# fabian-sp/GGLasso

Hardware: AMD Instinct MI355X
Metric: ADMM iters/sec on (K=32,p=500) GGL at 1/2/4/8 GPUs; eigh HBM GB/s vs peak (higher is better)
Workload: dtype f64

## Files before the change

### gglasso_amd/_lib.py

```python
import ctypes
import os

import numpy as np

_HERE = os.path.dirname(os.path.abspath(__file__))
LIB_PATH = os.path.join(_HERE, "lib", "libggl_hip.so")
DEV_LIB_PATH = os.path.join(_HERE, "lib", "libggl_hip_dev.so")

REG_SGL, REG_GGL, REG_FGL, REG_FSGL = 0, 1, 2, 3
EIG_AUTO, EIG_JACOBI, EIG_ROCSOLVER, EIG_NEWTON_SCHULZ = 0, 1, 2, 3
CTX_STREAM_GIVEN = 1 << 16
OPTIONS = {"speculate": 1, "spec_factor": 2, "ns_mode": 3, "ns_degrees": 4, "theta_flat": 5, "rank_eig": 6, "parts": 7,
           "parts_max_tiles": 8, "symm_variant": 9, "spin_wait": 10, "fused_bounds": 11, "pipeline": 12, "fused_start": 13, "parts_small": 14, "ns_tol": 15, "cw_warm": 16, "chain": 17, "rank_l0_coarse": 18, "isolate": 19, "rank_deflate": 20, "rank_l0_deflate": 21, "fused_cw": 22, "omega_lds": 23, "early_part": 24, "part_priority": 25, "fused_w": 26, "rank_cw": 27, "bound_side": 28, "lds_pinned": 29, "join_flag": 30, "cw_rider": 31, "copy_rider": 32, "reduce_rider": 33, "parts_bias": 34, "parts_order": 35, "download_threads": 36, "group_sched": 37, "omega_poly": 38}


def eig_flags(method=EIG_AUTO, ns_mode=0, ns_degrees=0):
    return int(method) | ((int(ns_mode) & 0x3) << 8) | ((int(ns_degrees) & 0xf) << 12)

JACOBI_MAX_P = 128
NS_MIN_P = 8
BUF_S, BUF_OMEGA, BUF_THETA, BUF_L, BUF_X, BUF_GROUPSQ, BUF_NORMS, BUF_OMEGA_PREV = range(8)
E_ARG, E_HIP, E_SOLVER, E_ALLOC, E_COMM = -1, -2, -3, -4, -5
COV_CENTER, COV_SCALE, COV_TILE32, COV_TILE64 = 1, 2, 4, 8
PHASES = ("form_W", "eig_omega", "recon_omega", "theta", "eig_L", "recon_L", "dual", "reduce", "eig_omega2", "bound",
# ... 89 lines not shown
    "ggl_finalize_L": ([_vp, _i, ctypes.POINTER(_i)], _i),
    "ggl_failed_instances": ([_vp, ctypes.POINTER(_i)], _i),
    "ggl_failed_reason": ([_vp, _i, _dp], _i),
    "ggl_debug_poison": ([_i], _i),
    "ggl_set_odd_dl": ([_i], _i),
    "ggl_reset_instance": ([_vp, _i], _i),
    "ggl_ctx_create_subset": ([_vp, ctypes.POINTER(_i), _i, ctypes.POINTER(_vp)], _i),
    "ggl_get_snapshot_k": ([_vp, _i, _dp, _dp], _i),
    "ggl_get_snapshot_state_k": ([_vp, _i, _dp, _dp], _i),
    "ggl_dev_ns_schedule": ([_d, _i, _i, ctypes.POINTER(_i), _dp, ctypes.POINTER(_i)], _i),
    "ggl_dev_ns_schedule_tol": ([_d, _i, _d, _i, ctypes.POINTER(_i), _dp, ctypes.POINTER(_i)], _i),
    "ggl_dev_group_partition": ([ctypes.POINTER(_i), _i, _i, _i, ctypes.POINTER(_i)], _i),
    "ggl_dev_ns_units": ([_d, _i, _d], _i),
    "ggl_dev_omega_poly_plan": ([_d, _d, _i, ctypes.POINTER(_i), _dp, ctypes.POINTER(_i)], _i),
    "ggl_omega_poly_stats": ([_vp, ctypes.POINTER(ctypes.c_longlong)], _i),
    "ggl_ns_stats": ([_vp, ctypes.POINTER(ctypes.c_longlong)], _i),
    "ggl_rank_stats": ([_vp, ctypes.POINTER(ctypes.c_longlong)], _i),
    "ggl_deflate_stats": ([_vp, ctypes.POINTER(ctypes.c_longlong)], _i),
    "ggl_finalize_stats": ([_vp, ctypes.POINTER(ctypes.c_longlong)], _i),
    "ggl_eig_info": ([_vp, ctypes.POINTER(_i)], _i),
    "ggl_last_dispatch": ([_vp, ctypes.POINTER(ctypes.c_longlong)], _i),
    "ggl_eigh_batched": ([_i, _i, _dp, _dp, _dp, _i], _i),
    "ggl_phiplus": ([_i, _i, _dp, _dp, _dp, _dp], _i),
    "ggl_prox_rank_norm": ([_i, _i, _dp, _dp, _dp, _dp], _i),
    "ggl_phiplus_matrix": ([_i, _i, _dp, _dp, _dp, _i], _i),
    "ggl_rank_matrix": ([_i, _i, _dp, _dp, _dp, _i], _i),
    "ggl_rank_matrix_ex": ([_i, _i, _dp, _dp, _dp, _i, _d, ctypes.POINTER(ctypes.c_longlong)], _i),
    "ggl_rank_matrix_deflate": ([_i, _i, _dp, _dp, _dp, _i, _d, ctypes.POINTER(ctypes.c_longlong)], _i),
    "ggl_prox_od_1norm": ([_i, _dp, _d, _dp, _dp], _i),
    "ggl_prox_p": ([_i, _i, _dp, _d, _d, _i, _dp], _i),
# ... 107 lines not shown
```

### gglasso_amd/build.py

```python
import os
import subprocess
import sys
from concurrent.futures import ThreadPoolExecutor

HERE = os.path.dirname(os.path.abspath(__file__))
CSRC = os.path.join(HERE, "csrc")
LIBDIR = os.path.join(HERE, "lib")
LIB = os.path.join(LIBDIR, "libggl_hip.so")
SOURCES = ["elementwise.hip", "theta_pair.hip", "theta_fsgl.hip", "ext_group.hip", "eig_jacobi.hip", "recon_gemm.hip", "gemm_sym.hip", "covariance.hip", "stars.hip", "kendall.hip", "gemm_i8.hip", "deflate.hip", "omega_lds.hip", "newton_schulz.hip", "ggl_comm.hip", "probes_dev.hip",
           "capi_ctx.hip", "capi_omega.hip", "capi_lstep.hip", "capi_batch.hip", "capi_snapshots.hip", "capi_checks.hip",
           "capi_stats.hip", "capi_comm.hip", "capi_ext.hip", "capi_ops.hip", "capi_data.hip"]
HEADERS = ["common.hpp", "kernels.hpp", "sym_tile.hpp", "ggl_comm.hpp", "capi_internal.hpp", os.path.join("..", "..", "include", "ggl_hip.h")]
HIPCC = os.environ.get("HIPCC", "/opt/rocm/bin/hipcc")
FLAGS = ["--offload-arch=gfx950", "-O3", "-std=c++17", "-fPIC", "-Wall", "-Wno-unused-function",
         "-mllvm", "-amdgpu-mfma-vgpr-form"]


def _stale(target, deps):
    if not os.path.exists(target):
        return True
    t = os.path.getmtime(target)
    return any(os.path.getmtime(d) > t for d in deps)


DEV_LIB = os.path.join(LIBDIR, "libggl_hip_dev.so")


# ... 36 lines not shown
```

### gglasso_amd/csrc/capi_ctx.hip

```cpp
#include "capi_internal.hpp"

static thread_local char g_err[512] = "";

int fail(int code, const char* fmt, ...)
{
    va_list ap;
    va_start(ap, fmt);
    vsnprintf(g_err, sizeof(g_err), fmt, ap);
    va_end(ap);
    return code;
}

void prof_collect(ggl_ctx* c)
{
    if (!c->prof_on) return;
    for (int ph = 0; ph < GGL_NPHASE; ++ph) {
        if (!c->ev_used[ph]) continue;
        float ms = 0.f;
        if (hipEventElapsedTime(&ms, c->ev[ph][0], c->ev[ph][1]) == hipSuccess) {
            c->ph_ms[ph] += ms;
            c->ph_cnt[ph] += 1;
        }
        c->ev_used[ph] = false;
    }
// ... 313 lines not shown
            if (v >= 0 && !symm_variant_built((int)v))
                return fail(GGL_E_ARG, "bad argument: product-kernel variant not in this build");
            c->symm_variant = (int)v;
            break;
        case GGL_OPT_SPIN_WAIT: c->spin_wait = v != 0.0; break;
        case GGL_OPT_FUSED_BOUNDS: c->fused_bounds = v != 0.0; break;
        case GGL_OPT_PIPELINE: c->pipeline = v != 0.0; break;
        case GGL_OPT_FUSED_START: c->fused_start = v != 0.0; break;
        case GGL_OPT_PARTS_SMALL: c->parts_small = (int)v; break;
        case GGL_OPT_GROUP_SCHED:
            if (v != 0.0 && v != 1.0 && v != 2.0 && v != 3.0 && v != 12.0 && v != 13.0)
                return fail(GGL_E_ARG, "bad argument: GGL_OPT_GROUP_SCHED is 0, 1, 2, 3, 12 or 13");
            c->group_sched = (int)v;
            break;
        case GGL_OPT_OMEGA_POLY:
            if (v != 0.0 && v != 1.0) return fail(GGL_E_ARG, "bad argument: GGL_OPT_OMEGA_POLY is 0 or 1");
            c->omega_poly = (int)v;
            break;
#ifdef GGL_DEV
        case GGL_OPT_PARTS_BIAS: c->parts_bias = (int)v; break;
        case GGL_OPT_PARTS_ORDER: c->parts_order = (int)v; break;
        case GGL_OPT_CHAIN: c->chain_mode = (v == 2.0) ? 2 : (v != 0.0 ? 1 : 0); break;
        case GGL_OPT_FUSED_CW: c->fused_cw = v != 0.0; break;
        case GGL_OPT_RANK_CW: c->rank_cw = v != 0.0; break;
        case GGL_OPT_BOUND_SIDE: c->bound_side = (int)v; break;
#else
        case GGL_OPT_PARTS_BIAS: case GGL_OPT_PARTS_ORDER: case GGL_OPT_CHAIN: case GGL_OPT_FUSED_CW: case GGL_OPT_RANK_CW:
        case GGL_OPT_BOUND_SIDE: case GGL_OPT_PART_PRIORITY:
            if (v == 0.0) break;
            return fail(GGL_E_ARG, "bad argument: option %d is a measured-and-rejected alternative that only the development "
                        "library (libggl_hip_dev.so, python -m gglasso_amd.build --dev) carries", opt);
// ... 474 lines not shown
```

### gglasso_amd/csrc/capi_internal.hpp

```cpp
#pragma once
#include <hip/hip_runtime.h>
#include <rocblas/rocblas.h>
#include <rocsolver/rocsolver.h>

#include <algorithm>
#include <cmath>
#include <cstdarg>
#include <cstdio>
#include <cstring>
#include <numeric>
#include <atomic>
#include <thread>
#include <mutex>
#include <chrono>
#include <vector>

#include "../../include/ggl_hip.h"
#include "kernels.hpp"
#include "ggl_comm.hpp"

using namespace ggl;


#define HIPCHK(expr)                                                                                   \
// ... 95 lines not shown
    unsigned long long* join_words = nullptr;
    unsigned long long join_seq = 0;
    hipEvent_t ev_bfork[MAX_PARTS] = {}, ev_bjoin[MAX_PARTS] = {};
    bool pipeline = true, pre_valid = false, pre_spec_pending = false;
    bool last_step_hint = false;
    double* pre_beta = nullptr;
    long long pre_launched = 0, pre_dropped = 0;
    int download_threads = 8;
    GGL_DEV_OPT(int, parts_order);
    GGL_DEV_OPT(int, parts_bias);
    int group_sched = 1;
    long long group_steps = 0;
    long long group_changes = 0;
    int last_groups = 1, last_group_len[MAX_PARTS] = {}, last_group_units[MAX_PARTS] = {};
    double group_units_sum[MAX_PARTS] = {};
    int omega_poly = 1;
    long long poly_seqs = 0, poly_seqs_total = 0;
    int poly_last_deg = 0;
    int parts_small = 8;
    bool fused_start = true;
    bool fused_bounds = true;
    bool lds_omega = true;
    int lds_waves = 0;
    double* lds_tab = nullptr;
    int lds_ntab = 0, lds_tab_deg = -1;
    double lds_lnq = 0.0, lds_tab_tol = -1.0;
    long long lds_calls = 0, lds_misses = 0;
    int lds_cool = 0, lds_cool_next = 4;
    bool lds_last = false;
    GGL_DEV_OPT(bool, fused_cw);
    int theta_flat = 2;
    bool state_symmetric = true;
    bool S_symmetric = false;
// ... 196 lines not shown
```

### gglasso_amd/csrc/capi_omega.hip

```cpp
#include "capi_internal.hpp"

int eig_recon(ggl_ctx* c, double* A, double* out, double* Dv, int map, const double* betaK, int ph_eig,
                     int ph_recon)
{
    c->info_dirty = true;
    if (use_jacobi(c)) {
        if (ph_eig >= 0) PB(c, ph_eig);
        HIPCHK(launch_jacobi(c->stream, A, Dv, nullptr, out, map, betaK, c->info, c->K, c->p));
        if (ph_eig >= 0) PE(c, ph_eig);
        return GGL_OK;
    }
    if (ph_eig >= 0) PB(c, ph_eig);
    {
        int rcb = blas_handle(c, &c->blas);
        if (rcb) return rcb;
    }
    if (c->use_syevj) {
        rocblas_status sj = rocsolver_dsyevj_strided_batched(c->blas, rocblas_esort_none, rocblas_evect_original,
                                                             rocblas_fill_upper, c->p, A, c->p,
                                                             (rocblas_stride)c->p * c->p, 0.0, c->E, 100,
                                                             (rocblas_int*)c->sweeps, Dv, c->p, c->info, c->K);
        if (sj != rocblas_status_success) return fail(GGL_E_SOLVER, "rocsolver_dsyevj_strided_batched: status %d", (int)sj);
        if (ph_eig >= 0) PE(c, ph_eig);
        if (ph_recon >= 0) PB(c, ph_recon);
// ... 196 lines not shown
    t.n += 1;
}
void trace_host(ggl_ctx* c, int tag)
{
    ggl_ctx::Trace& t = c->trace;
    if (!t.on || t.nhost >= t.cap) return;
    t.host_us[t.nhost] = std::chrono::duration<double, std::micro>(std::chrono::steady_clock::now() - t.t0).count();
    t.host_tag[t.nhost] = tag;
    t.nhost += 1;
}
void trace_symm_hook(hipStream_t st, int kind, void* arg) { trace_mark((ggl_ctx*)arg, st, 10 + kind); }

static void note_family(ggl_ctx* c, const NsPlan& pl)
{
    c->poly_seqs_total += 1;
    if (pl.direct) { c->poly_seqs += 1; c->poly_last_deg = pl.direct; }
}

static int omega_groups(const ggl_ctx* c, const double* cb, const double* beta_h, int K, int* Kh, int* k0h, int* gunits)
{
    if (!c->group_sched || K < 2 || c->ns_force == 2 || c->chain_mode || c->comm) return 1;
    {
        const double I = 2.5e-14 * (double)c->p * c->p * c->p, F = 6.5e-6;
        if (c->group_sched < 10 && (double)K * 1e-7 > 0.01 * 7.0 * (F + K * I)) return 1;
    }
    std::vector<int> u(K);
    for (int k = 0; k < K; ++k) {
        double ck = cb[k] * (1.0 + 1e-10);
        if (!(ck > 0.0) || !std::isfinite(ck) || !(beta_h[k] > 0.0)) return 1;
        if (ck < 4.0 * beta_h[k]) ck = 4.0 * beta_h[k];
        u[k] = ns_units_query(std::sqrt(4.0 * beta_h[k] / ck), c->ns_degrees, c->ns_tol);
// ... 1020 lines not shown
```

### gglasso_amd/csrc/capi_ops.hip

```cpp
#include "capi_internal.hpp"

static int eig_common(int K, int p, const double* A, const double* beta, double* D, double* Q, double* out, int map,
                      int eig_method)
{
    ARGCHK(K >= 1 && p >= 1 && A, "K, p, A");
    ARGCHK(eig_method != GGL_EIG_JACOBI || jacobi_fits(p), "GGL_EIG_JACOBI needs p <= GGL_JACOBI_MAX_P");
    const bool jac = (eig_method == GGL_EIG_JACOBI) || (eig_method == GGL_EIG_AUTO && jacobi_fits(p));
    const size_t n = (size_t)K * p * p, kp = (size_t)K * p;
    DevBuf dA, dD, dR, dO, dB, dE, dS;
    int* dinfo = nullptr;
    HIPCHK(dA.alloc(n));
    HIPCHK(dD.alloc(kp));
    HIPCHK(dB.alloc(K));
    HIPCHK(hipMalloc(&dinfo, K * sizeof(int)));
    struct InfoFree { int* p; ~InfoFree() { (void)hipFree(p); } } infofree{dinfo};
    UP(dA.p, A, n);
    if (beta) UP(dB.p, beta, K);
    if (out) HIPCHK(dO.alloc(n));
    std::vector<int> info(K);
    if (jac) {
        if (Q) HIPCHK(dR.alloc(n));
        HIPCHK(launch_jacobi(nullptr, dA.p, dD.p, dR.p, dO.p, map, beta ? dB.p : nullptr, dinfo, K, p));
        HIPCHK(hipDeviceSynchronize());
        HIPCHK(hipMemcpy(info.data(), dinfo, K * sizeof(int), hipMemcpyDeviceToHost));
// ... 710 lines not shown
    return n;
}

extern "C" int ggl_dev_group_partition(const int* units, int K, int p, int max_groups, int* len_out)
{
    ARGCHK(units && len_out && K >= 1 && p >= 1 && max_groups >= 1 && max_groups <= 3, "units, len_out, K, p, 1 <= max_groups <= 3");
    return ns_group_partition(units, K, p, max_groups, len_out);
}
extern "C" int ggl_dev_ns_units(double l, int degrees, double tol) { return ns_units_query(l, degrees, tol); }
extern "C" int ggl_dev_omega_poly_plan(double a, double tol, int degrees, int* deg, double* out, int* units)
{
    ARGCHK(deg && out && units && a > 0.0 && a < 1.0, "deg, out, units, 0 < a < 1");
    return ns_poly_query(std::sqrt(a), degrees, tol, deg, out, units, out + 16, out + 17);
}

extern "C" int ggl_dev_ns_schedule_tol(double l, int degrees, double tol, int max_steps, int* deg_out, double* coef_out,
                                       int* units_out)
{
    ARGCHK(deg_out && coef_out && units_out, "output pointers");
    ARGCHK(l > 0.0 && l <= 1.0, "l must be in (0,1]");
    ARGCHK(tol >= 0.0 && tol <= 1e-6, "tol in [0, 1e-6]");
    const int n = ns_schedule_query(l, degrees, max_steps, deg_out, coef_out, units_out, std::max(tol, NS_TOL_EXACT));
    if (n < 0) return fail(GGL_E_ARG, "no schedule within %d steps", max_steps);
    return n;
}

#ifdef GGL_DEV
extern "C" int ggl_dev_coissue_probe(double* out12)
{
    ARGCHK(out12, "out");
// ... 276 lines not shown
```

### gglasso_amd/csrc/capi_stats.hip

```cpp
#include "capi_internal.hpp"

extern "C" int ggl_scale_X(ggl_ctx* c, double factor)
{
    ARGCHK(c, "ctx");
    HIPCHK(hipSetDevice(c->device));
    DROP_PRE(c);
    launch_scale(c->stream, c->X, factor, c->n);
    HIPCHK(hipGetLastError());
    return GGL_OK;
}

extern "C" int ggl_profile_enable(ggl_ctx* c, int on)
{
    ARGCHK(c, "ctx");
    HIPCHK(hipSetDevice(c->device));
    if (on && !c->ev[0][0]) {
        for (int ph = 0; ph < GGL_NPHASE; ++ph)
            for (int e = 0; e < 2; ++e) HIPCHK(hipEventCreate(&c->ev[ph][e]));
        for (int q = 0; q < 2; ++q)
            for (int e = 0; e < 2; ++e) HIPCHK(hipEventCreate(&c->ev_early[q][e]));
    }
    c->prof_on = (on == 2) ? 2 : (on != 0 ? 1 : 0);
    return GGL_OK;
}
// ... 19 lines not shown
    out[13] = c->last_variant;
    out[14] = c->ns_eigh_fallbacks;
    out[15] = c->pre_dropped;
    return GGL_OK;
}

extern "C" int ggl_omega_poly_stats(ggl_ctx* c, long long out[3])
{
    ARGCHK(c && out, "ctx, out");
    out[0] = c->poly_seqs;
    out[1] = c->poly_seqs_total;
    out[2] = c->poly_last_deg;
    return GGL_OK;
}

extern "C" int ggl_group_stats(ggl_ctx* c, long long out[11], double* units_sum)
{
    ARGCHK(c && out, "ctx, out");
    out[10] = c->group_changes;
    out[0] = c->group_steps;
    out[1] = c->last_groups;
    for (int g = 0; g < 4; ++g) {
        out[2 + g] = c->last_groups > 1 ? c->last_group_len[g] : 0;
        out[6 + g] = c->last_groups > 1 ? c->last_group_units[g] : 0;
        if (units_sum) units_sum[g] = c->group_units_sum[g];
    }
    return GGL_OK;
}

extern "C" int ggl_spectral_bounds(ggl_ctx* c, double* c_out, double* beta_out)
// ... 154 lines not shown
```

### gglasso_amd/csrc/kernels.hpp

```cpp
#pragma once
#include <hip/hip_runtime.h>
#include <stddef.h>

#define GGL_NNORM 5

namespace ggl {

enum EigMap {
    MAP_PHIPLUS = 0,
    MAP_RANK = 1,
    MAP_IDENT = 2
};

int elementwise_blocks(int p);
void launch_form_W(hipStream_t st, double* W, const double* Theta, const double* L, const double* X,
                   const double* S, const double* betaK, int K, int p);
void launch_theta_sgl(hipStream_t st, double* Theta, double* X, double* C, const double* Omega,
                      const double* OmegaPrev, const double* L, const double* l1K,
                      const double* mask, const double* invrhoK, int latent, double* partials, int K, int p, const int* skip = nullptr,
                      const int* pk = nullptr, size_t mask_stride = 0);
void launch_dual_update(hipStream_t st, double* X, const double* Omega, const double* OmegaPrev,
                        const double* Theta, const double* L, double* partials, int K, int p);
void launch_reduce_partials(hipStream_t st, const double* partials, int K, int nblk, int nv, double* out,
                            unsigned long long* seq = nullptr, unsigned long long seq_val = 0, unsigned* arrive = nullptr);
// ... 237 lines not shown
void symm_set_rider(const CwRider& r);
void symm_flush_rider(hipStream_t st);
void symm_set_launch_hook(void (*fn)(hipStream_t, int, void*), void* arg);
void launch_symm_pair(hipStream_t st, const double* A, const double* B, double* C, const double* A1, const double* B1,
                      double* C1, const double* coef2K, int K, int p, int variant);

static constexpr double NS_TOL_EXACT = 4e-16;
static constexpr double NS_TOL_DEFAULT = 2e-12;
static constexpr int NS_MAX_STEPS = 24;
static constexpr int NS_RANK_MAX_STEPS = 40;
static constexpr int NS_MAX_LAUNCHES = 2 * NS_RANK_MAX_STEPS + 1 + 3;
static inline size_t NS_SLOT(int K) { return (size_t)K * 2 * NS_NCOEF; }
static constexpr double NS_SYM_KAPPA_MAX = 300.0;
static constexpr double NS_KAPPA_LIMIT = 1e12;
struct NsPlan {
    int steps = 0; int products = 0; bool stable = false; double kappa = 0.0; int units = 0; int direct = 0;
    double check = 5e-5;
    unsigned char deg[NS_RANK_MAX_STEPS] = {};
};
int form_W_tiles(int p);
void launch_form_W_sym(hipStream_t st, double* W, const double* Theta, const double* L, const double* X,
                       const double* S, const double* betaK, int K, int p);
int ns_plan(const double* cbound_h, const double* beta_h, int K, double* coef_h, double* start_h, NsPlan* plan,
            int force_mode, int degrees = 9, double tol = NS_TOL_EXACT, int poly = 0);
int ns_poly_query(double l, int degrees, double tol, int* deg, double* coef, int* units, double* a_out, double* err_out);
int ns_schedule_query(double l, int degrees, int max_steps, int* deg, double* coef, int* units, double tol = NS_TOL_EXACT);
int ns_units_query(double l, int degrees, double tol);
int ns_group_partition(const int* units, int K, int p, int max_groups, int* len_out);
void ns_prepare(hipStream_t st, const double* pre0_d, const double* pre1_d, const double* W, double* Ap, double* Bp,
                int K, int p, int variant, double* start2 = nullptr, double* rowpart = nullptr, double* fropart = nullptr,
                bool start_w = false);
void ns_run(hipStream_t st, const NsPlan& plan, const double* coef_d, const double* start_d, const double* W,
            double* AB, double* YP, double* Tb, double* out, int K, int p, int variant, size_t pstride = 0,
            bool fused_start = false, hipEvent_t bprime_free = nullptr);
int ns_chain_ops(const NsPlan& plan, const double* pre0_d, const double* pre1_d, const double* coef_d, const double* W,
                 double* AB, double* YP, double* NX, double* Tb, double* out, int K, int p, size_t pstride, double* start2,
                 double* rowpart, double* fropart, SymmOp* ops, int max_ops);
double* ns_fused_start(const NsPlan& plan, const double* start_hk, double* YP, double* Tb, size_t n1, double* row);

int norm_bounds_blocks(int p);
// ... 46 lines not shown
```

### gglasso_amd/csrc/newton_schulz.hip

```cpp
#include <cmath>
#include <vector>
#include <unordered_map>

#include <functional>
#include "common.hpp"
#include "kernels.hpp"

namespace ggl {

static constexpr int FT = 32, FTY = 8, FQ = FT / FTY;

template <bool HAS_L>
__global__ __launch_bounds__(256) void k_form_W_sym(double* __restrict__ W, const double* __restrict__ Theta,
                                                    const double* __restrict__ L, const double* __restrict__ X,
                                                    const double* __restrict__ S, const double* __restrict__ betaK,
                                                    int p)
{
    __shared__ double tile[FT][FT + 1];
    const int k = blockIdx.y;
    const int T = (p + FT - 1) / FT;
    int I = 0, b = blockIdx.x;
    while (b >= T - I) { b -= T - I; ++I; }
    const int J = I + b;
    const int I0 = I * FT, J0 = J * FT;
// ... 455 lines not shown
}

int ns_poly_query(double l, int degrees, double tol, int* deg, double* coef, int* units, double* a_out, double* err_out)
{
    if (!(l > 0.0) || !(l <= 1.0)) return -1;
    const NsPoly pp = ns_poly_plan(l, tol);
    const int chosen = ns_poly_choice(l, degrees, tol);
    *deg = pp.deg;
    for (int j = 0; j <= NS_POLY_MAXDEG; ++j) coef[j] = j <= pp.deg ? pp.co[j] : 0.0;
    *units = pp.deg ? pp.units : -1;
    if (a_out) *a_out = pp.a;
    if (err_out) *err_out = pp.err;
    return chosen ? 1 : 0;
}

int ns_schedule_query(double l, int degrees, int max_steps, int* deg, double* coef, int* units, double tol)
{
    if (!(l > 0.0) || !(l <= 1.0)) return -1;
    const NsSeq& sq = (degrees >= 100) ? ns_sign_schedule(l, degrees - 100, tol) : ns_mixed_schedule(l, degrees, tol);
    if (sq.n < 1 || sq.n > max_steps || sq.cost >= (1 << 29)) return -1;
    for (int i = 0; i < sq.n; ++i) {
        deg[i] = sq.deg[i];
        for (int j = 0; j < 5; ++j) coef[6 * i + j] = sq.st[i].t[j];
        coef[6 * i + 5] = sq.st[i].lnew;
    }
    *units = (degrees >= 100) ? sq.cost : 2 + sq.cost;
    return sq.n;
}

int ns_units_query(double l, int degrees, double tol)
// ... 92 lines not shown
{
    std::vector<double> c(K);
    double kappa = 1.0;
    for (int k = 0; k < K; ++k) {
        c[k] = cbound_h[k] * (1.0 + 1e-10);
        if (!(c[k] > 0.0) || !std::isfinite(c[k]) || !(beta_h[k] > 0.0)) return -1;
        if (c[k] < 4.0 * beta_h[k]) c[k] = 4.0 * beta_h[k];
        kappa = std::fmax(kappa, c[k] / (4.0 * beta_h[k]));
    }
    const bool stable = (force_mode == 2) || (force_mode == 0 && kappa > NS_SYM_KAPPA_MAX);
    if (kappa > NS_KAPPA_LIMIT) return -2;
    const double lmin = 1.0 / std::sqrt(kappa);
    plan->stable = stable;
    plan->kappa = kappa;
    plan->direct = 0;
    auto put = [&](int g, int k, double cI, double cAcc, double cE, double dI = 0.0, double dC = 0.0, double dE = 0.0,
                   double cE2 = 0.0, double dE2 = 0.0) {
        double* o = coef_h + (size_t)g * NS_SLOT(K) + (size_t)k * NS_NCOEF;
        o[0] = cI; o[1] = cAcc; o[2] = cE; o[3] = dI; o[4] = dC; o[5] = dE; o[6] = cE2; o[7] = dE2;
    };
    const int pd = (!stable && poly) ? ns_poly_choice(lmin, degrees, tol) : 0;
    if (pd) {
        const NsPoly pp = ns_poly_plan(lmin, tol, pd);
        const int J = pd / 3;
        const double a = pp.a, m = 0.5 * (1.0 + a), h = 0.5 * (1.0 - a), u = 1.0 / (h * h * h);
        plan->direct = pd;
        plan->steps = 1;
        plan->deg[0] = 0;
        plan->units = pp.units;
        plan->products = J + 2;
        for (int k = 0; k < K; ++k) {
            const double ck = c[k], hc = 0.5 * std::sqrt(ck);
            auto digit = [&](int j, double* o3) {
                const double a0 = pp.co[3 * j], a1 = pp.co[3 * j + 1], a2 = pp.co[3 * j + 2];
                o3[0] = a0 - a1 * (m / h) + a2 * (m / h) * (m / h);
                o3[1] = a1 / (ck * h) - 2.0 * a2 * m / (ck * h * h);
// ... 124 lines not shown
}

void ns_run(hipStream_t st, const NsPlan& plan, const double* coef_d, const double* start_d, const double* W,
            double* AB, double* YP, double* Tb, double* out, int K, int p, int variant, size_t pstride, bool fused_start,
            hipEvent_t bprime_free)
{
    bool bwaited = bprime_free == nullptr;
    const double* bprime = AB + (pstride ? pstride : (size_t)K * p * p);
    auto before_write = [&](const double* o1, const double* o2) {
        if (!bwaited && (o1 == bprime || o2 == bprime)) { (void)hipStreamWaitEvent(st, bprime_free, 0); bwaited = true; }
    };
    struct AtExit { std::function<void()> f; ~AtExit() { f(); } } at_exit{[&]() { before_write(bprime, nullptr); }};
    const size_t cs = NS_SLOT(K), n1 = pstride ? pstride : (size_t)K * p * p;
    const int n = plan.steps;
    int g = 0;
    if (plan.direct) {
        if (!fused_start) launch_ns_start(st, Tb, nullptr, AB, AB + n1, W, start_d, K, p, 4);
        const int J = plan.direct / 3;
        auto hbuf = [&](int j) { return (j & 1) ? YP + n1 : out; };
        launch_symm(st, AB, AB + n1, YP, hbuf(J - 1), AB + n1, coef_d + cs * g++, K, p, variant, nullptr, nullptr, nullptr, AB);
        for (int j = J - 2; j >= 1; --j)
            launch_symm(st, hbuf(j + 1), YP, hbuf(j), nullptr, AB + n1, coef_d + cs * g++, K, p, variant, nullptr, nullptr,
                        nullptr, AB);
        launch_symm(st, hbuf(1), YP, out, nullptr, Tb, coef_d + cs * g++, K, p, variant);
        return;
    }
    double *cur = YP, *nxt = AB;
    if (plan.deg[0] >= 5 && !plan.stable) {
        if (plan.deg[0] == 5) {
            if (!fused_start)
// ... 49 lines not shown
    if (plan.stable || (plan.deg[0] < 5 && !plan.direct) || !start2) return 0;
    const size_t cs = NS_SLOT(K), n1 = pstride ? pstride : (size_t)K * p * p;
    const int n = plan.steps;
    int no = 0, g = 0;
    bool ok = true;
    auto add = [&](const double* A, const double* B, double* C, double* C2, const double* E, const double* coef,
                   double* rp = nullptr, double* fp = nullptr) -> SymmOp* {
        if (no >= max_ops) { ok = false; return nullptr; }
        SymmOp& o = ops[no++];
        o = SymmOp{};
        o.A = A; o.B = B; o.C = C; o.C2 = C2; o.E = E; o.coef = coef; o.rowpart = rp; o.fropart = fp;
        return &o;
    };
    double* Ap = AB;
    double* Bp = AB + n1;
    if (plan.direct) {
        const int J = plan.direct / 3;
        auto hbuf = [&](int j) { return (j & 1) ? YP + n1 : out; };
        add(W, W, Ap, nullptr, nullptr, pre0_d);
        SymmOp* o = add(Ap, Ap, Bp, start2, Ap, pre1_d, rowpart, fropart);
        if (o) o->E2 = W;
        o = add(Ap, Bp, YP, hbuf(J - 1), Bp, coef_d + cs * g++);
        if (o) o->E2 = Ap;
        for (int j = J - 2; j >= 1; --j) {
            o = add(hbuf(j + 1), YP, hbuf(j), nullptr, Bp, coef_d + cs * g++);
            if (o) o->E2 = Ap;
        }
        add(hbuf(1), YP, out, nullptr, start2, coef_d + cs * g++);
        (void)NX;
        return ok ? no : 0;
// ... 569 lines not shown
```

### gglasso_amd/solver.py

```python
import math
import time
import warnings

import numpy as np

from . import _lib
from ._lib import as_c, check, ptr

_REG = {"SGL": _lib.REG_SGL, "GGL": _lib.REG_GGL, "FGL": _lib.REG_FGL, "FSGL": _lib.REG_FSGL}


ENGINE_OPTIONS = {}


RANK_REL_TOL = 1e-9


def latent_rank(L, rel_tol=0.0):
    a = np.abs(np.linalg.eigvalsh(L))
    return int(np.count_nonzero(a > a.max() * max(rel_tol, L.shape[0] * np.finfo(np.float64).eps)))


def _host_period(A, K=None, p=None):
    if K is not None:
# ... 449 lines not shown
        ms = np.zeros(len(_lib.PHASES))
        cnt = (ctypes.c_longlong * len(_lib.PHASES))()
        check(self.lib.ggl_profile_read(self.h, ptr(ms), cnt, int(reset)))
        return {name: (float(ms[i]), int(cnt[i])) for i, name in enumerate(_lib.PHASES)}

    def ns_stats(self):
        import ctypes
        out = (ctypes.c_longlong * 16)()
        check(self.lib.ggl_ns_stats(self.h, out))
        return dict(zip(("calls", "steps", "stable_calls", "units", "launches", "rank_calls", "rank_retries",
                         "rank_fallbacks", "rank_launches", "spec_calls", "spec_misses", "spin_timeouts", "last_parts",
                         "last_variant", "eigh_fallbacks", "pre_dropped"), (int(v) for v in out)))

    def poly_stats(self):
        import ctypes
        out = (ctypes.c_longlong * 3)()
        check(self.lib.ggl_omega_poly_stats(self.h, out))
        return dict(zip(("seqs", "seqs_total", "last_deg"), (int(v) for v in out)))

    def rank_stats(self):
        import ctypes
        out = (ctypes.c_longlong * 4)()
        check(self.lib.ggl_rank_stats(self.h, out))
        st = dict(zip(("calls", "continued_calls", "continued_instances", "eigh_fallbacks"), (int(v) for v in out)))
        d = (ctypes.c_longlong * 2)()
        check(self.lib.ggl_deflate_stats(self.h, d))
        st["deflated_calls"], st["deflated_instances"] = int(d[0]), int(d[1])
        return st

    def group_stats(self):
        import ctypes
        out = (ctypes.c_longlong * 11)()
        us = np.zeros(4)
# ... 422 lines not shown
```

### include/ggl_hip.h

```cpp
#ifndef GGL_HIP_H
#define GGL_HIP_H

#ifdef __cplusplus
extern "C" {
#endif

#define GGL_VERSION 300

#define GGL_OK 0
#define GGL_E_ARG (-1)
#define GGL_E_HIP (-2)
#define GGL_E_SOLVER (-3)
#define GGL_E_ALLOC (-4)
#define GGL_E_COMM (-5)

#define GGL_REG_SGL 0
#define GGL_REG_GGL 1
#define GGL_REG_FGL 2
#define GGL_REG_FSGL 3

#define GGL_EIG_AUTO 0
#define GGL_EIG_JACOBI 1
#define GGL_EIG_ROCSOLVER 2
#define GGL_EIG_NEWTON_SCHULZ 3
// ... 168 lines not shown
#define GGL_PH_EIG_L 4
#define GGL_PH_RECON_L 5
#define GGL_PH_DUAL 6
#define GGL_PH_REDUCE 7
#define GGL_PH_EIG_OMEGA2 8
#define GGL_PH_BOUND 9
#define GGL_PH_ALLREDUCE_GROUPSQ 10
#define GGL_PH_ALLREDUCE_NORMS 11
#define GGL_NPHASE 12
int ggl_profile_enable(ggl_ctx *ctx, int on);
int ggl_profile_read(ggl_ctx *ctx, double ms[GGL_NPHASE], long long count[GGL_NPHASE], int reset);
int ggl_ns_stats(ggl_ctx *ctx, long long out[16]);
int ggl_lds_stats(ggl_ctx *ctx, long long out[4]);
int ggl_group_stats(ggl_ctx *ctx, long long out[11], double *units_sum);
int ggl_omega_poly_stats(ggl_ctx *ctx, long long out[3]);
int ggl_spectral_bounds(ggl_ctx *ctx, double *c_out, double *beta_out);
int ggl_pipeline_stats(ggl_ctx *ctx, long long out[10]);
int ggl_rank_stats(ggl_ctx *ctx, long long out[4]);
int ggl_deflate_stats(ggl_ctx *ctx, long long out[2]);
int ggl_finalize_stats(ggl_ctx *ctx, long long out[2]);
int ggl_last_dispatch(ggl_ctx *ctx, long long out[4]);
int ggl_fsgl_stats(ggl_ctx *ctx, long long out[4]);
int ggl_trace_start(ggl_ctx *ctx, int max_events);
int ggl_trace_read(ggl_ctx *ctx, double *out, int cap);
int ggl_eig_info(ggl_ctx *ctx, int *out);

int ggl_dev_symm(int K, int p, const double *A, const double *B, const double *E, const double *coef5K,
                 double *C, double *C2, int variant);
int ggl_dev_symm_bench(int K, int p, int variant, int iters, double *ms_out);
int ggl_dev_omega_lds(int K, int p, const double *Theta, const double *L, const double *X, const double *S, const double *beta,
                      double tol, int degrees, double *Omega, double *cbound, int iters, double *out);
int ggl_dev_symm_bounds(int K, int p, const double *A, const double *B, int variant, double *C,
                        double *rowsum_out, double *fro2_out, double *bound_out);
int ggl_dev_ns_schedule(double l, int degrees, int max_steps, int *deg_out, double *coef_out, int *units_out);
int ggl_dev_ns_schedule_tol(double l, int degrees, double tol, int max_steps, int *deg_out, double *coef_out,
                            int *units_out);
int ggl_dev_group_partition(const int *units, int K, int p, int max_groups, int *len_out);
int ggl_dev_ns_units(double l, int degrees, double tol);
int ggl_dev_omega_poly_plan(double a, double tol, int degrees, int *deg, double *out, int *units);
#ifdef GGL_DEV
int ggl_dev_i8_stages(int n);
int ggl_dev_symm_i8(int K, int p, int S, int dmax, const double *A, const double *B, double scaleA, double scaleB, double *C,
                    int iters, double *ms_out);
int ggl_dev_omega_i8(int K, int p, const double *W, const double *beta, const double *cbound, const int *cfg5, double tol,
                     double *Omega, int iters, double *ms_out);
int ggl_dev_mfma_f64_peak(double *tflops_out);
int ggl_dev_coissue_probe(double *out12);
int ggl_dev_mfma_lds_probe(double *out6);
int ggl_dev_chain_run(int K, int p, int nprod, int iters, double *out);
int ggl_dev_switch_bench(int K, int p, int variant, int iters, int mode, double *ms_out);
int ggl_dev_vendor_bench(int K, int p, int mode, int iters, double *ms_out);
int ggl_dev_fill_copy_probe(int reps, int K, int p, int slices, int gap_us, long long out[2]);
int ggl_dev_symm_timeline(int K, int p, long long *out, int max_blocks, int *nblocks_out);
int ggl_dev_chain_probe(int K, int p, int variant, int nprod, int iters, int two_level, double *out);
// ... 44 lines not shown
```

Measured before the change: 1487.

## Add precomputed degree-24 polynomial family for Omega Newton-Schulz step, enabled by default

Adds a table of precomputed polynomial coefficient sets, keyed by quantised spectral bound, that evaluates the matrix-function approximation for the Omega update in a fixed chain of four symmetric-product launches. The family is chosen when its launch count beats both the mixed Newton-Schulz schedule and the direct polynomial, and the option now defaults to 2 so it runs by default. It aims to cut the number of matrix products per ADMM iteration. It only applies to a narrow band of quantised bounds in the table, and its accuracy depends on the tabulated error bounds.

```diff
diff --git a/gglasso_amd/_lib.py b/gglasso_amd/_lib.py
--- a/gglasso_amd/_lib.py
+++ b/gglasso_amd/_lib.py
@@ -127,6 +127,8 @@
     "ggl_dev_ns_units": ([_d, _i, _d], _i),
     "ggl_dev_omega_poly_plan": ([_d, _d, _i, ctypes.POINTER(_i), _dp, ctypes.POINTER(_i)], _i),
     "ggl_omega_poly_stats": ([_vp, ctypes.POINTER(ctypes.c_longlong)], _i),
+    "ggl_omega_family_stats": ([_vp, ctypes.POINTER(ctypes.c_longlong)], _i),
+    "ggl_dev_omega_family_plan": ([_d, _d, _i, ctypes.POINTER(_i), _dp, _dp, _dp, ctypes.POINTER(_i)], _i),
     "ggl_ns_stats": ([_vp, ctypes.POINTER(ctypes.c_longlong)], _i),
     "ggl_rank_stats": ([_vp, ctypes.POINTER(ctypes.c_longlong)], _i),
     "ggl_deflate_stats": ([_vp, ctypes.POINTER(ctypes.c_longlong)], _i),
diff --git a/gglasso_amd/build.py b/gglasso_amd/build.py
--- a/gglasso_amd/build.py
+++ b/gglasso_amd/build.py
@@ -10,7 +10,7 @@
 SOURCES = ["elementwise.hip", "theta_pair.hip", "theta_fsgl.hip", "ext_group.hip", "eig_jacobi.hip", "recon_gemm.hip", "gemm_sym.hip", "covariance.hip", "stars.hip", "kendall.hip", "gemm_i8.hip", "deflate.hip", "omega_lds.hip", "newton_schulz.hip", "ggl_comm.hip", "probes_dev.hip",
            "capi_ctx.hip", "capi_omega.hip", "capi_lstep.hip", "capi_batch.hip", "capi_snapshots.hip", "capi_checks.hip",
            "capi_stats.hip", "capi_comm.hip", "capi_ext.hip", "capi_ops.hip", "capi_data.hip"]
-HEADERS = ["common.hpp", "kernels.hpp", "sym_tile.hpp", "ggl_comm.hpp", "capi_internal.hpp", os.path.join("..", "..", "include", "ggl_hip.h")]
+HEADERS = ["common.hpp", "kernels.hpp", "sym_tile.hpp", "ggl_comm.hpp", "capi_internal.hpp", "ns_family_tables.hpp", os.path.join("..", "..", "include", "ggl_hip.h")]
 HIPCC = os.environ.get("HIPCC", "/opt/rocm/bin/hipcc")
 FLAGS = ["--offload-arch=gfx950", "-O3", "-std=c++17", "-fPIC", "-Wall", "-Wno-unused-function",
          "-mllvm", "-amdgpu-mfma-vgpr-form"]
diff --git a/gglasso_amd/csrc/capi_ctx.hip b/gglasso_amd/csrc/capi_ctx.hip
--- a/gglasso_amd/csrc/capi_ctx.hip
+++ b/gglasso_amd/csrc/capi_ctx.hip
@@ -351,7 +351,7 @@
             c->group_sched = (int)v;
             break;
         case GGL_OPT_OMEGA_POLY:
-            if (v != 0.0 && v != 1.0) return fail(GGL_E_ARG, "bad argument: GGL_OPT_OMEGA_POLY is 0 or 1");
+            if (v != 0.0 && v != 1.0 && v != 2.0) return fail(GGL_E_ARG, "bad argument: GGL_OPT_OMEGA_POLY is 0, 1 or 2");
             c->omega_poly = (int)v;
             break;
 #ifdef GGL_DEV
diff --git a/gglasso_amd/csrc/capi_internal.hpp b/gglasso_amd/csrc/capi_internal.hpp
--- a/gglasso_amd/csrc/capi_internal.hpp
+++ b/gglasso_amd/csrc/capi_internal.hpp
@@ -133,9 +133,11 @@
     long long group_changes = 0;
     int last_groups = 1, last_group_len[MAX_PARTS] = {}, last_group_units[MAX_PARTS] = {};
     double group_units_sum[MAX_PARTS] = {};
-    int omega_poly = 1;
+    int omega_poly = 2;
     long long poly_seqs = 0, poly_seqs_total = 0;
     int poly_last_deg = 0;
+    long long fam_seqs = 0;
+    int fam_last_products = 0;
     int parts_small = 8;
     bool fused_start = true;
     bool fused_bounds = true;
diff --git a/gglasso_amd/csrc/capi_omega.hip b/gglasso_amd/csrc/capi_omega.hip
--- a/gglasso_amd/csrc/capi_omega.hip
+++ b/gglasso_amd/csrc/capi_omega.hip
@@ -234,7 +234,9 @@
 static void note_family(ggl_ctx* c, const NsPlan& pl)
 {
     c->poly_seqs_total += 1;
-    if (pl.direct) { c->poly_seqs += 1; c->poly_last_deg = pl.direct; }
+    if (pl.direct) c->poly_seqs += 1;
+    if (pl.family) { c->fam_seqs += 1; c->fam_last_products = pl.products; }
+    else if (pl.direct) c->poly_last_deg = pl.direct;
 }
 
 static int omega_groups(const ggl_ctx* c, const double* cb, const double* beta_h, int K, int* Kh, int* k0h, int* gunits)
diff --git a/gglasso_amd/csrc/capi_ops.hip b/gglasso_amd/csrc/capi_ops.hip
--- a/gglasso_amd/csrc/capi_ops.hip
+++ b/gglasso_amd/csrc/capi_ops.hip
@@ -748,6 +748,13 @@
     return ns_poly_query(std::sqrt(a), degrees, tol, deg, out, units, out + 16, out + 17);
 }
 
+extern "C" int ggl_dev_omega_family_plan(double a, double tol, int degrees, int* wiring, double* rows, double* last,
+                                         double* info, int* taken)
+{
+    ARGCHK(wiring && rows && last && info && taken && a > 0.0 && a < 1.0, "wiring, rows, last, info, taken, 0 < a < 1");
+    return ns_family_query(std::sqrt(a), degrees, tol, wiring, rows, last, info, taken);
+}
+
 extern "C" int ggl_dev_ns_schedule_tol(double l, int degrees, double tol, int max_steps, int* deg_out, double* coef_out,
                                        int* units_out)
 {
diff --git a/gglasso_amd/csrc/capi_stats.hip b/gglasso_amd/csrc/capi_stats.hip
--- a/gglasso_amd/csrc/capi_stats.hip
+++ b/gglasso_amd/csrc/capi_stats.hip
@@ -57,6 +57,15 @@
     return GGL_OK;
 }
 
+extern "C" int ggl_omega_family_stats(ggl_ctx* c, long long out[3])
+{
+    ARGCHK(c && out, "ctx, out");
+    out[0] = c->fam_seqs;
+    out[1] = c->poly_seqs_total;
+    out[2] = c->fam_last_products;
+    return GGL_OK;
+}
+
 extern "C" int ggl_group_stats(ggl_ctx* c, long long out[11], double* units_sum)
 {
     ARGCHK(c && out, "ctx, out");
diff --git a/gglasso_amd/csrc/kernels.hpp b/gglasso_amd/csrc/kernels.hpp
--- a/gglasso_amd/csrc/kernels.hpp
+++ b/gglasso_amd/csrc/kernels.hpp
@@ -275,7 +275,7 @@
 static constexpr double NS_SYM_KAPPA_MAX = 300.0;
 static constexpr double NS_KAPPA_LIMIT = 1e12;
 struct NsPlan {
-    int steps = 0; int products = 0; bool stable = false; double kappa = 0.0; int units = 0; int direct = 0;
+    int steps = 0; int products = 0; bool stable = false; double kappa = 0.0; int units = 0; int direct = 0; int family = 0;
     double check = 5e-5;
     unsigned char deg[NS_RANK_MAX_STEPS] = {};
 };
@@ -285,6 +285,7 @@
 int ns_plan(const double* cbound_h, const double* beta_h, int K, double* coef_h, double* start_h, NsPlan* plan,
             int force_mode, int degrees = 9, double tol = NS_TOL_EXACT, int poly = 0);
 int ns_poly_query(double l, int degrees, double tol, int* deg, double* coef, int* units, double* a_out, double* err_out);
+int ns_family_query(double l, int degrees, double tol, int* wiring, double* rows, double* last, double* info, int* taken);
 int ns_schedule_query(double l, int degrees, int max_steps, int* deg, double* coef, int* units, double tol = NS_TOL_EXACT);
 int ns_units_query(double l, int degrees, double tol);
 int ns_group_partition(const int* units, int K, int p, int max_groups, int* len_out);
diff --git a/gglasso_amd/csrc/newton_schulz.hip b/gglasso_amd/csrc/newton_schulz.hip
--- a/gglasso_amd/csrc/newton_schulz.hip
+++ b/gglasso_amd/csrc/newton_schulz.hip
@@ -5,6 +5,7 @@
 #include <functional>
 #include "common.hpp"
 #include "kernels.hpp"
+#include "ns_family_tables.hpp"
 
 namespace ggl {
 
@@ -493,6 +494,48 @@
     return chosen ? 1 : 0;
 }
 
+static constexpr double NS_FAM_EVAL = 2e-14;
+
+static const NsFamCell* ns_family_cell(double l, double tol)
+{
+    const double t = std::fmin(std::fmax(tol, NS_TOL_EXACT), 1e-6);
+    if (!(l > 0.0) || !(l < 1.0) || t <= 2.0 * NS_FAM_EVAL) return nullptr;
+    const NsKey q = ns_quantise(l);
+    for (const NsFamCell& cell : NS_FAM_CELLS)
+        if (cell.key == q.key)
+            return (std::fabs(cell.a - q.l * q.l) <= 1e-12 && cell.err + NS_FAM_EVAL <= t) ? &cell : nullptr;
+    return nullptr;
+}
+
+static const NsFamCell* ns_family_choice(double l, int degrees, double tol, int pd)
+{
+    if (!(l > 0.0) || !(l < 1.0) || 1.0 / (l * l) > NS_SYM_KAPPA_MAX) return nullptr;
+    const NsFamCell* cell = ns_family_cell(l, tol);
+    if (!cell) return nullptr;
+    const NsSeq& sq = ns_mixed_schedule(l, degrees, tol);
+    const int ns_units = (sq.n < 1 || sq.cost >= (1 << 29)) ? (1 << 30) : 2 + sq.cost;
+    const int other = std::min(ns_units, pd ? pd / 3 + 2 : (1 << 30));
+    return 2 + NS_FAM_LAUNCHES < other ? cell : nullptr;
+}
+
+int ns_family_query(double l, int degrees, double tol, int* wiring, double* rows, double* last, double* info, int* taken)
+{
+    if (!(l > 0.0) || !(l <= 1.0)) return -1;
+    *taken = 0;
+    const NsKey q = ns_quantise(l);
+    const NsFamCell* cell = nullptr;
+    for (const NsFamCell& c : NS_FAM_CELLS) if (c.key == q.key) cell = &c;
+    if (!cell) return 0;
+    for (int t = 0; t < NS_FAM_LAUNCHES; ++t) {
+        for (int j = 0; j < 4; ++j) wiring[4 * t + j] = NS_FAM_WIRE[t][j];
+        if (t < NS_FAM_LAUNCHES - 1) for (int j = 0; j < NS_NCOEF; ++j) rows[NS_NCOEF * t + j] = cell->row[t][j];
+    }
+    for (int j = 0; j < 5; ++j) last[j] = cell->last[j];
+    info[0] = cell->a; info[1] = cell->err; info[2] = NS_FAM_EVAL;
+    *taken = ns_family_choice(l, degrees, tol, ns_poly_choice(l, degrees, tol)) != nullptr;
+    return NS_FAM_LAUNCHES;
+}
+
 int ns_schedule_query(double l, int degrees, int max_steps, int* deg, double* coef, int* units, double tol)
 {
     if (!(l > 0.0) || !(l <= 1.0)) return -1;
@@ -615,12 +658,36 @@
     plan->stable = stable;
     plan->kappa = kappa;
     plan->direct = 0;
+    plan->family = 0;
     auto put = [&](int g, int k, double cI, double cAcc, double cE, double dI = 0.0, double dC = 0.0, double dE = 0.0,
                    double cE2 = 0.0, double dE2 = 0.0) {
         double* o = coef_h + (size_t)g * NS_SLOT(K) + (size_t)k * NS_NCOEF;
         o[0] = cI; o[1] = cAcc; o[2] = cE; o[3] = dI; o[4] = dC; o[5] = dE; o[6] = cE2; o[7] = dE2;
     };
     const int pd = (!stable && poly) ? ns_poly_choice(lmin, degrees, tol) : 0;
+    if (const NsFamCell* fc = (!stable && poly >= 2) ? ns_family_choice(lmin, degrees, tol, pd) : nullptr) {
+        plan->direct = NS_FAM_DEGREE;
+        plan->family = NS_FAM_LAUNCHES;
+        plan->steps = 1;
+        plan->deg[0] = 0;
+        plan->units = plan->products = 2 + NS_FAM_LAUNCHES;
+        for (int k = 0; k < K; ++k) {
+            const double ck = c[k], hc = 0.5 * std::sqrt(ck);
+            auto cp = [&](int id) { return id == 0 ? 1.0 / ck : (id == 1 ? 1.0 / (ck * ck) : 1.0); };
+            double* s = start_h + (size_t)k * 5;
+            s[0] = hc * fc->last[2] / ck; s[1] = hc * fc->last[3] / (ck * ck); s[2] = hc * fc->last[1]; s[3] = 0.0; s[4] = 0.0;
+            int g = 0;
+            for (int t = 0; t < NS_FAM_LAUNCHES - 1; ++t) {
+                const unsigned char* w = NS_FAM_WIRE[t];
+                const double* r = fc->row[t];
+                put(g++, k, r[0], r[1] * cp(w[0]) * cp(w[1]), r[2] * cp(w[2]), r[3], r[4], r[5] * cp(w[2]), r[6] * cp(w[3]),
+                    r[7] * cp(w[3]));
+            }
+            const unsigned char* w = NS_FAM_WIRE[NS_FAM_LAUNCHES - 1];
+            put(g++, k, 0.0, hc * fc->last[0] * cp(w[0]) * cp(w[1]), 1.0, 0.0, 0.0, 0.0, hc * fc->last[4] * cp(w[3]), 0.0);
+        }
+        return 0;
+    }
     if (pd) {
         const NsPoly pp = ns_poly_plan(lmin, tol, pd);
         const int J = pd / 3;
@@ -775,6 +842,22 @@
     const size_t cs = NS_SLOT(K), n1 = pstride ? pstride : (size_t)K * p * p;
     const int n = plan.steps;
     int g = 0;
+    if (plan.family) {
+        if (!fused_start) launch_ns_start(st, Tb, nullptr, AB, AB + n1, W, start_d, K, p, 4);
+        double* slot[5] = {AB, AB + n1, YP, YP + n1, out};
+        const double* sm[2 + 2 * NS_FAM_LAUNCHES] = {AB, AB + n1};
+        for (int t = 0; t < NS_FAM_LAUNCHES; ++t) {
+            const unsigned char* w = NS_FAM_WIRE[t];
+            const bool last = t == NS_FAM_LAUNCHES - 1;
+            double* C = last ? out : slot[NS_FAM_SLOT_RUN[t][0]];
+            double* C2 = (last || NS_FAM_SLOT_RUN[t][1] == 255) ? nullptr : slot[NS_FAM_SLOT_RUN[t][1]];
+            before_write(C, C2);
+            launch_symm(st, sm[w[0]], sm[w[1]], C, C2, last ? Tb : sm[w[2]], coef_d + cs * g++, K, p, variant, nullptr, nullptr,
+                        nullptr, sm[w[3]]);
+            if (!last) { sm[2 + 2 * t] = C; sm[3 + 2 * t] = C2; }
+        }
+        return;
+    }
     if (plan.direct) {
         if (!fused_start) launch_ns_start(st, Tb, nullptr, AB, AB + n1, W, start_d, K, p, 4);
         const int J = plan.direct / 3;
@@ -854,6 +937,23 @@
     };
     double* Ap = AB;
     double* Bp = AB + n1;
+    if (plan.family) {
+        double* slot[7] = {nullptr, nullptr, YP, YP + n1, out, NX, NX + n1};
+        const double* sm[2 + 2 * NS_FAM_LAUNCHES] = {Ap, Bp};
+        add(W, W, Ap, nullptr, nullptr, pre0_d);
+        SymmOp* o = add(Ap, Ap, Bp, start2, Ap, pre1_d, rowpart, fropart);
+        if (o) o->E2 = W;
+        for (int t = 0; t < NS_FAM_LAUNCHES; ++t) {
+            const unsigned char* w = NS_FAM_WIRE[t];
+            const bool last = t == NS_FAM_LAUNCHES - 1;
+            double* C = last ? out : slot[NS_FAM_SLOT_CHAIN[t][0]];
+            double* C2 = (last || NS_FAM_SLOT_CHAIN[t][1] == 255) ? nullptr : slot[NS_FAM_SLOT_CHAIN[t][1]];
+            o = add(sm[w[0]], sm[w[1]], C, C2, last ? start2 : sm[w[2]], coef_d + cs * g++);
+            if (o) o->E2 = sm[w[3]];
+            if (!last) { sm[2 + 2 * t] = C; sm[3 + 2 * t] = C2; }
+        }
+        return ok ? no : 0;
+    }
     if (plan.direct) {
         const int J = plan.direct / 3;
         auto hbuf = [&](int j) { return (j & 1) ? YP + n1 : out; };
diff --git a/gglasso_amd/csrc/ns_family_tables.hpp b/gglasso_amd/csrc/ns_family_tables.hpp
--- /dev/null
+++ b/gglasso_amd/csrc/ns_family_tables.hpp
@@ -0,0 +1,45 @@
+#pragma once
+
+static constexpr int NS_FAM_LAUNCHES = 4;
+static constexpr int NS_FAM_DEGREE = 24;
+static constexpr unsigned char NS_FAM_WIRE[4][4] = {{0, 1, 1, 0}, {2, 3, 3, 0}, {4, 5, 5, 0}, {6, 7, 1, 4}};
+static constexpr unsigned char NS_FAM_SLOT_RUN[3][2] = {{2, 3}, {1, 4}, {2, 3}};
+static constexpr unsigned char NS_FAM_SLOT_CHAIN[3][2] = {{2, 3}, {5, 4}, {2, 3}};
+struct NsFamCell { int key; double a, err; double row[3][8]; double last[5]; };
+static constexpr NsFamCell NS_FAM_CELLS[] = {
+    {999946, 0x1.b9b17ddb3857fp-2, 0x1.0e32133e2ddfcp-38,
+     {{-0x1.8d7ece41959f4p+0, 0x1.0000000000000p+0, -0x1.21d306832c97ap+2, -0x1.fafb6d9c554b1p+0, 0x1.7dc258ac721bfp-1, -0x1.03ce70e43daf4p+2, 0x1.aad4ef1c79baep+2, 0x1.a0f97ab9b43a7p+2},
+      {0x1.daafa1dc66349p+0, 0x1.0000000000000p+0, 0x1.2bb4014006d98p-2, 0x1.f449745671294p-2, 0x1.22f55a6a8eb0cp-5, -0x1.b7467733e0be5p-3, 0x1.95c52ce0da855p-1, 0x1.542e1c16b4d75p-2},
+      {0x1.797dca4c5aeccp-4, 0x1.0000000000000p+0, 0x1.cfc7c4f8fbc73p-4, 0x1.48e19dda2234cp-1, 0x1.289110e609d60p-4, 0x1.8ec911f6ae08ap-2, -0x1.50f69105fb7b7p-5, -0x1.e559ada475e60p-3}},
+     {-0x1.e8b2a3099ad17p-8, 0x1.1c93bda8f9778p-2, 0x1.14d5521683f9bp+0, -0x1.1d0c7657878dap-2, -0x1.2a52bb13aa997p-7}},
+    {999945, 0x1.c2cac3c1e7ec3p-2, 0x1.d09f444f54debp-39,
+     {{-0x1.a6a4bca71df8ap+0, 0x1.0000000000000p+0, -0x1.1b1ff6abcdbc1p+2, -0x1.e860167746ea3p+0, 0x1.ac597a70ea188p-1, -0x1.09052610c5c9fp+2, 0x1.a4cc4d3574849p+2, 0x1.98c31f80a3f3cp+2},
+      {0x1.da3f047e69c6bp+0, 0x1.0000000000000p+0, 0x1.d43b943cea94fp-3, 0x1.c8fde09108d7fp-2, 0x1.18650c603d6c4p-5, -0x1.8a1865f7db207p-3, 0x1.81f5dd3896c3bp-1, 0x1.48873e76244d5p-2},
+      {0x1.d127ee1af7adfp-5, 0x1.0000000000000p+0, 0x1.5f2d6c74b19e3p-3, 0x1.5ed631353abfdp-1, 0x1.1af74ab0308a7p-4, 0x1.2c6d966a37fa1p-2, -0x1.10422cb65165dp-4, -0x1.c29022fc51b61p-3}},
+     {-0x1.ebda5baf5b955p-8, 0x1.22b5f14de9dcap-2, 0x1.0d8403e8737f2p+0, -0x1.10c6c11535edcp-2, -0x1.1b1e430a3cc0fp-7}},
+    {999944, 0x1.cbcd6b407139bp-2, 0x1.e800d14848f46p-39,
+     {{-0x1.9caa8143fdac3p+0, 0x1.0000000000000p+0, -0x1.1cebff6b54f30p+2, -0x1.732b7a794ab3ap+0, 0x1.7d895b4efdaf0p-1, -0x1.a64698a8ba422p+1, 0x1.adda0494e0192p+2, 0x1.4cc2bbb225739p+2},
+      {0x1.e23b36502297cp+0, 0x1.0000000000000p+0, 0x1.47fb917d38e34p-2, 0x1.fc5a589a3bfb4p-2, 0x1.20975ee6a9490p-5, -0x1.bd65e55a9b9e5p-3, 0x1.88d0ec9c325dfp-1, 0x1.18a0b40c480eep-2},
+      {0x1.3534649dc73e3p-4, 0x1.0000000000000p+0, 0x1.3992ed5b0aa80p-3, 0x1.3dc2a3531a406p-1, 0x1.62684faae46e7p-4, 0x1.4eada43a63343p-2, -0x1.f5f3f0701c310p-5, -0x1.63e2a3a6c8360p-2}},
+     {-0x1.415b5521ab6d3p-7, 0x1.20c073dd0c148p-2, 0x1.1512b48c85566p+0, -0x1.19187bdb7ec19p-2, -0x1.49ef413779552p-7}},
+    {999943, 0x1.d4b900b5851bap-2, 0x1.41b1046d2a164p-41,
+     {{-0x1.f376bd7f2ce30p+0, 0x1.0000000000000p+0, -0x1.1e6c2180c6258p+2, -0x1.d9652ea50133fp+1, 0x1.fb401e9b2d58cp-1, -0x1.dd292ba13da91p+2, 0x1.ac339e849a63fp+2, 0x1.645098ab48283p+3},
+      {0x1.c1cfc6cb7e9d4p+0, 0x1.0000000000000p+0, 0x1.1a73dfdcc24e4p-4, 0x1.7c38466f040fep-2, 0x1.8c9bcdd4a1299p-6, -0x1.0167930959ba5p-3, 0x1.68577d79d1368p-1, 0x1.9a48f963c8bcbp-2},
+      {-0x1.41f5d72471d4bp-7, 0x1.0000000000000p+0, 0x1.779c9b4097576p-3, 0x1.6d6edfdf91f9ap-1, 0x1.0209d75af3fb9p-5, 0x1.0ab373b67bc86p-2, -0x1.a1bcbc8b09e2bp-4, -0x1.00512032a6dd0p-5}},
+     {-0x1.0165cd7cd0044p-8, 0x1.2bc04464e69aap-2, 0x1.f7e3747d37976p-1, -0x1.f54ff03844468p-3, -0x1.4dddcfb53b377p-8}},
+    {999942, 0x1.dd8d1baa5aa68p-2, 0x1.3d102efe4b02dp-41,
+     {{-0x1.0a1875a41fe06p+1, 0x1.0000000000000p+0, -0x1.1b5d9ae2cc106p+2, -0x1.56e86325afeb4p+2, 0x1.0663332b44a23p+0, -0x1.4fcfad06d9784p+3, 0x1.a8494bef957c5p+2, 0x1.f1ae42637e25bp+3},
+      {0x1.ae060e9b7d2ebp+0, 0x1.0000000000000p+0, -0x1.b2eacf2756b09p-6, 0x1.40c5c97a5c19bp-2, 0x1.2e5de26530937p-6, -0x1.74aed6d023321p-4, 0x1.4ef5010f85299p-1, 0x1.b5e2a2414f0b3p-2},
+      {-0x1.4f3f8e9370a8ep-5, 0x1.0000000000000p+0, 0x1.5792283f00cd7p-3, 0x1.724f033c9625bp-1, 0x1.7bbc4a7793c75p-6, 0x1.c407786dfad93p-3, -0x1.0404a6a84f19ep-3, -0x1.f57c6024b89e4p-7}},
+     {-0x1.97391c6c3679fp-9, 0x1.33256d20dc8dep-2, 0x1.e7adbf216fcd4p-1, -0x1.dda56fdef3cabp-3, -0x1.f8b46159eb33cp-9}},
+    {999941, 0x1.e6495e422c4cdp-2, 0x1.0c66888dad5dap-41,
+     {{-0x1.0c91e295f0984p+1, 0x1.0000000000000p+0, -0x1.1e9cd835f84e7p+2, -0x1.2fd5615cd2d75p+2, 0x1.fffe8326b3498p-1, -0x1.24c377bc79065p+3, 0x1.b1834093d9243p+2, 0x1.b8e725da50a73p+3},
+      {0x1.bab06bac7b116p+0, 0x1.0000000000000p+0, 0x1.75a09121484d1p-9, 0x1.591c058a98641p-2, 0x1.3d9ea8abf2d9bp-6, -0x1.9ced8eb4e6b7fp-4, 0x1.5c179d22c5228p-1, 0x1.ae5a218c15c97p-2},
+      {-0x1.7282a69d35820p-8, 0x1.0000000000000p+0, 0x1.73b544a7cc7d7p-3, 0x1.6bdb49d0cf1e3p-1, 0x1.8dbba2327662dp-6, 0x1.d05c301e1b1f6p-3, -0x1.a12a38985886fp-4, -0x1.d8717a399be75p-6}},
+     {-0x1.b3aa5f8889067p-9, 0x1.324a543b97b8cp-2, 0x1.e9d97799a06d6p-1, -0x1.dc3a8c4815b51p-3, -0x1.0c6db0ce82866p-8}},
+    {999940, 0x1.eeed74aff9c9fp-2, 0x1.c10bb3581f410p-42,
+     {{-0x1.20203e9e20c61p+1, 0x1.0000000000000p+0, -0x1.204aeee7aace2p+2, -0x1.96896b637ab6bp+2, 0x1.ff446f76b9beep-1, -0x1.7fabcdca7664fp+3, 0x1.b7d5844e88ffap+2, 0x1.1fd53dc1c308ap+4},
+      {0x1.ab2d5c0f45d2fp+0, 0x1.0000000000000p+0, -0x1.79f6ea1c96ba3p-5, 0x1.41d4776f96f0ap-2, 0x1.fb48b9af8c886p-7, -0x1.46c8a7e1c2c91p-4, 0x1.468efe7b88432p-1, 0x1.b5e80e88a44adp-2},
+      {-0x1.0d7df04f9ea3dp-5, 0x1.0000000000000p+0, 0x1.56963a1ace3afp-3, 0x1.6f8f76b826775p-1, 0x1.2bb8b0b325c7dp-6, 0x1.bcfcf96d54598p-3, -0x1.efe294fb47d50p-4, -0x1.d590fa1e7ca9fp-8}},
+     {-0x1.4f09218b289edp-9, 0x1.3714986b91fcap-2, 0x1.dfa7684ed3550p-1, -0x1.cda97e5dee880p-3, -0x1.a237b083a7141p-9}},
+};
diff --git a/gglasso_amd/solver.py b/gglasso_amd/solver.py
--- a/gglasso_amd/solver.py
+++ b/gglasso_amd/solver.py
@@ -487,9 +487,11 @@
 
     def poly_stats(self):
         import ctypes
-        out = (ctypes.c_longlong * 3)()
+        out, fam = (ctypes.c_longlong * 3)(), (ctypes.c_longlong * 3)()
         check(self.lib.ggl_omega_poly_stats(self.h, out))
-        return dict(zip(("seqs", "seqs_total", "last_deg"), (int(v) for v in out)))
+        check(self.lib.ggl_omega_family_stats(self.h, fam))
+        return dict(zip(("seqs", "seqs_total", "last_deg", "family_seqs", "family_products"),
+                        (int(out[0]), int(out[1]), int(out[2]), int(fam[0]), int(fam[2]))))
 
     def rank_stats(self):
         import ctypes
diff --git a/include/ggl_hip.h b/include/ggl_hip.h
--- a/include/ggl_hip.h
+++ b/include/ggl_hip.h
@@ -206,6 +206,7 @@
 int ggl_lds_stats(ggl_ctx *ctx, long long out[4]);
 int ggl_group_stats(ggl_ctx *ctx, long long out[11], double *units_sum);
 int ggl_omega_poly_stats(ggl_ctx *ctx, long long out[3]);
+int ggl_omega_family_stats(ggl_ctx *ctx, long long out[3]);
 int ggl_spectral_bounds(ggl_ctx *ctx, double *c_out, double *beta_out);
 int ggl_pipeline_stats(ggl_ctx *ctx, long long out[10]);
 int ggl_rank_stats(ggl_ctx *ctx, long long out[4]);
@@ -230,6 +231,7 @@
 int ggl_dev_group_partition(const int *units, int K, int p, int max_groups, int *len_out);
 int ggl_dev_ns_units(double l, int degrees, double tol);
 int ggl_dev_omega_poly_plan(double a, double tol, int degrees, int *deg, double *out, int *units);
+int ggl_dev_omega_family_plan(double a, double tol, int degrees, int *wiring, double *rows, double *last, double *info, int *taken);
 #ifdef GGL_DEV
 int ggl_dev_i8_stages(int n);
 int ggl_dev_symm_i8(int K, int p, int S, int dmax, const double *A, const double *B, double scaleA, double scaleB, double *C,
```

After: 1480. Within noise of the previous version (-0.5%).
